# rrwick/Filtlong

Measured on NVIDIA H100. Metric: Gbases/sec scored+filtered, higher is better.
Workload: dtype f64

## Files before the change

### filtlong_b200/csrc/fl_phred.cu

```cuda
#include "fl_device.cuh"

namespace {

#define PH_THREADS 256
#define PH_SMEM (256 * 8 * 16 + 256 * 16 * 8)
#define PH_SEG 16384
#define PH_LONG (PH_SEG + PH_SEG / 2)

#define ITEM_FUSED 0xFFFFFFFFu
#define ITEM_MEAN 0xFFFFFFFEu

struct Tab {
    const double2 *tqa;
    const double *ta;
};

struct PhredArgs {
    const uint8_t *qual;
    const uint64_t *off;
    const int32_t *len;
    uint32_t n;
    const double *lut;
    fl_params p;
    int32_t *r_len, *r_first, *r_last, *r_nbad, *r_nchild;
    double *r_mean, *r_window;
    uint8_t *r_passed;
    unsigned long long *r_rowstart;
    uint32_t *w_parent;
    int32_t *w_start, *w_end;
    double *w_mean, *w_window;
    uint8_t *w_passed;
    unsigned long long read_base, row_base;
    const unsigned long long *item_start;
    const uint32_t *order;
    const uint2 *items;
    unsigned long long n_items;
    double *it_a, *it_b, *it_c;
    uint32_t *fallback;
    unsigned long long *work;
    unsigned long long *phred_paths;
    int head_len;
};

__device__ __forceinline__ unsigned byte_of(uint32_t w, int i) { return (w >> (8 * i)) & 0xFFu; }

template <int WI>
__device__ __forceinline__ void out_words(const uint4 &a, const uint4 &b, unsigned sh, uint32_t ow[4]) {
    const uint32_t c[8] = {a.x, a.y, a.z, a.w, b.x, b.y, b.z, b.w};
#pragma unroll
    for (int k = 0; k < 4; ++k) ow[k] = __funnelshift_r(c[WI + k], c[WI + k + 1], sh);
}

template <bool DO_SUM, bool DO_WIN>
__device__ __forceinline__ void step(unsigned cin, unsigned cout, const Tab &t, double &sum, double &w, double &best) {
    if (DO_SUM && DO_WIN) {
        const double2 qa = t.tqa[cin * 8];
        const double ao = t.ta[cout * 16];
        sum += qa.x;
        w -= ao;
        w += qa.y;
        if (w < best) best = w;
    } else if (DO_SUM) {
        sum += t.tqa[cin * 8].x;
    } else {
        const double ai = t.ta[cin * 16];
        const double ao = t.ta[cout * 16];
        w -= ao;
        w += ai;
        if (w < best) best = w;
    }
}

template <bool DO_SUM, bool DO_WIN>
__device__ __forceinline__ void chain(const uint8_t *__restrict__ q, int jlo, int jhi, int ws, const Tab &t, double &sum,
                                      double &w, double &best) {
    int j = jlo;
    for (; (j & 15) && j < jhi; ++j) step<DO_SUM, DO_WIN>(q[j], DO_WIN ? q[j - ws] : 0u, t, sum, w, best);
    if (j + 16 <= jhi) {
        const uint4 *qv = reinterpret_cast<const uint4 *>(q);
        const uint4 zero = make_uint4(0u, 0u, 0u, 0u);
        int blk = 0;
        unsigned sh = 0, wi = 0;
        uint4 oa = zero, ob = zero;
        if (DO_WIN) {
            const int i0 = j - ws;
            blk = i0 >> 4;
            sh = ((unsigned)i0 & 3u) * 8u;
            wi = ((unsigned)i0 & 15u) >> 2;
            oa = __ldg(qv + blk);
            ob = __ldg(qv + blk + 1);
        }
        uint4 in = __ldg(qv + (j >> 4));
        while (j + 16 <= jhi) {
            const bool more = j + 32 <= jhi;
            const uint4 in_next = more ? __ldg(qv + (j >> 4) + 1) : zero;
            const uint4 oc = (DO_WIN && more) ? __ldg(qv + blk + 2) : zero;
            uint32_t ow[4] = {0u, 0u, 0u, 0u};
            if (DO_WIN) {
                switch (wi) {
                    case 0: out_words<0>(oa, ob, sh, ow); break;
                    case 1: out_words<1>(oa, ob, sh, ow); break;
                    case 2: out_words<2>(oa, ob, sh, ow); break;
                    default: out_words<3>(oa, ob, sh, ow); break;
                }
            }
            const uint32_t iw[4] = {in.x, in.y, in.z, in.w};
#pragma unroll
            for (int k = 0; k < 4; ++k)
#pragma unroll
                for (int b = 0; b < 4; ++b)
                    step<DO_SUM, DO_WIN>(byte_of(iw[k], b), byte_of(ow[k], b), t, sum, w, best);
            in = in_next;
            oa = ob;
            ob = oc;
            ++blk;
            j += 16;
        }
    }
    for (; j < jhi; ++j) step<DO_SUM, DO_WIN>(q[j], DO_WIN ? q[j - ws] : 0u, t, sum, w, best);
}

__device__ __forceinline__ void write_read(const PhredArgs &a, uint32_t r, int L, double mean, double window) {
    const uint8_t passed = fl_hard_cutoffs(a.p, L, mean, window);
    a.r_len[r] = L;
    a.r_mean[r] = mean;
    a.r_window[r] = window;
    a.r_passed[r] = passed;
    a.r_first[r] = -1;
    a.r_last[r] = -1;
    a.r_nbad[r] = 0;
    a.r_nchild[r] = 0;
    a.r_rowstart[r] = a.row_base + r;
    a.w_parent[r] = (uint32_t)(a.read_base + r);
    a.w_start[r] = 0;
    a.w_end[r] = L;
    a.w_mean[r] = mean;
    a.w_window[r] = window;
    a.w_passed[r] = passed;
}

__device__ __forceinline__ void finish(const PhredArgs &a, uint32_t r, int L, double sum, double best) {
    const double wsd = (double)a.p.window_size;
    if (best < 0.5 / wsd) best = 0.0;
    write_read(a, r, L, 100.0 * sum / (double)L, 100.0 * best);
}

__device__ __forceinline__ void score_fused(const PhredArgs &a, uint32_t r, const Tab &t) {
    const int L = a.len[r], ws = a.p.window_size;
    const uint8_t *q = a.qual + a.off[r];
    double sum = 0.0, w = 0.0, best = 0.0;
    chain<true, false>(q, 0, L < ws ? L : ws, ws, t, sum, w, best);
    if (L <= ws) {
        const double mean = 100.0 * sum / (double)L;
        write_read(a, r, L, mean, mean);
        return;
    }
    w = sum / (double)ws;
    best = w;
    chain<true, true>(q, ws, L, ws, t, sum, w, best);
    finish(a, r, L, sum, best);
}

__device__ __forceinline__ int n_segments(int L, int ws) { return (L - ws + PH_SEG - 1) / PH_SEG; }

__device__ __forceinline__ unsigned long long items_of(int L, int ws) {
    if (L <= PH_LONG || L <= ws + PH_SEG) return 1ull;
    return 1ull + (unsigned long long)n_segments(L, ws);
}

__device__ __forceinline__ void score_segment(const PhredArgs &a, uint32_t r, int seg, size_t idx, const Tab &t) {
    const int L = a.len[r], ws = a.p.window_size;
    const uint8_t *q = a.qual + a.off[r];
    double sum = 0.0, w = 0.0, best = 0.0;
    chain<true, false>(q, 0, ws, ws, t, sum, w, best);
    const double w0 = sum / (double)ws;
    const int P = ws + seg * PH_SEG;
    const int Pend = (P + PH_SEG < L) ? P + PH_SEG : L;
    double entry = w0;
    if (seg > 0) {
        int e = 0;
        (void)frexp(w0, &e);
        const double scale = ldexp(1.0, 53 - e);
        long long s0 = 0, sp = 0;
        for (int i = 0; i < ws; ++i) {
            s0 += __double2ll_rn(t.ta[(unsigned)q[i] * 16] * scale);
            sp += __double2ll_rn(t.ta[(unsigned)q[P - ws + i] * 16] * scale);
        }
        entry = w0 + (double)(sp - s0) / scale;
    }
    w = entry;
    best = __longlong_as_double(0x7FF0000000000000ll);
    chain<false, true>(q, P, Pend, ws, t, sum, w, best);
    a.it_a[idx] = entry;
    a.it_b[idx] = w;
    a.it_c[idx] = best;
}

__device__ __forceinline__ Tab make_tables(const double *lut, unsigned char *smem_raw) {
    double2 *tqa_all = reinterpret_cast<double2 *>(smem_raw);
    double *ta_all = reinterpret_cast<double *>(smem_raw + 256 * 8 * 16);
    for (int i = threadIdx.x; i < 256 * 8; i += blockDim.x) {
        const int c = i >> 3;
        tqa_all[i] = make_double2(lut[c], lut[256 + c]);
    }
    for (int i = threadIdx.x; i < 256 * 16; i += blockDim.x) ta_all[i] = lut[256 + (i >> 4)];
    __syncthreads();
    const unsigned lane = threadIdx.x & 31;
    Tab t;
    t.tqa = tqa_all + (lane & 7);
    t.ta = ta_all + (lane & 15);
    return t;
}

__global__ void __launch_bounds__(PH_THREADS, 3) k_phred_items(PhredArgs a) {
    extern __shared__ __align__(16) unsigned char smem_raw[];
    const Tab t = make_tables(a.lut, smem_raw);
    const size_t T = (size_t)gridDim.x * blockDim.x;
    for (size_t it = (size_t)blockIdx.x * blockDim.x + threadIdx.x; it < a.n_items; it += T) {
        const size_t idx = a.order[it];
        const uint2 item = a.items[idx];
        const uint32_t r = item.x;
        if (item.y == ITEM_FUSED) {
            score_fused(a, r, t);
        } else if (item.y == ITEM_MEAN) {
            continue;
        } else {
            score_segment(a, r, (int)item.y, idx, t);
        }
    }
}

#define PH_MEAN_SMEM (256 * 16 * 8)
#define PH_MEAN_TILE 2048

__device__ __forceinline__ double serial_tile(const uint8_t *__restrict__ q, int lo, int hi, const double *__restrict__ qtab,
                                              double s) {
    for (int j = lo; j < hi; ++j) s += __ldg(qtab + (unsigned)q[j]);
    return s;
}

__global__ void __launch_bounds__(256) k_phred_mean_long(PhredArgs a, unsigned long long tie_binades) {
    extern __shared__ __align__(16) unsigned char smem_raw[];
    double *qtab_all = reinterpret_cast<double *>(smem_raw);
    for (int i = threadIdx.x; i < 256 * 16; i += blockDim.x) {
        const double v = a.lut[i >> 4];
        qtab_all[i] = (v >= 0.0 && v < 1.0) ? v : __longlong_as_double(0x7FF8000000000000ll);
    }
    __syncthreads();
    const unsigned lane = threadIdx.x & 31;
    const double *qtab = qtab_all + (lane & 15);
    const size_t warp = ((size_t)blockIdx.x * blockDim.x + threadIdx.x) >> 5, n_warps = ((size_t)gridDim.x * blockDim.x) >> 5;
    for (size_t r = warp; r < a.n; r += n_warps) {
        const size_t base = a.item_start[r];
        if (a.item_start[r + 1] - base <= 1) continue;
        const int L = a.len[r];
        const uint8_t *q = a.qual + a.off[r];
        const uint4 *qv = reinterpret_cast<const uint4 *>(q);
        double s = 0.0;
        int j = 0, small_left = 0;
        while (j < L) {
            int e = -2000;
            if (s > 0.0) {
                (void)frexp(s, &e);
                e -= 1;
            }
            const bool big = e >= 10 && e <= 1000 && small_left == 0;
            const bool lattice_ok = big || (e >= 6 && e <= 1000);
            const int T = big ? PH_MEAN_TILE : 128;
            const int hi = (j + T < L) ? j + T : L;
            bool done = false;
            if (lattice_ok) {
                const double C = ldexp(1.0, e), half_ulp = ldexp(1.0, e - 53);
                const bool check_ties = e < 64 && ((tie_binades >> e) & 1ull);
                double d = 0.0;
                unsigned bad = 0u;
#pragma unroll
                for (int c4 = 0; c4 < 4; ++c4) {
                    const int lo = j + 512 * c4 + 16 * (int)lane;
                    if (lo < hi) {
                        const uint4 v = __ldg(qv + (lo >> 4));
                        const uint32_t wv[4] = {v.x, v.y, v.z, v.w};
                        if (lo + 16 <= hi && !check_ties) {
#pragma unroll
                            for (int k = 0; k < 16; ++k) {
                                const double x = qtab[byte_of(wv[k >> 2], k & 3) * 16];
                                d += (C + x) - C;
                            }
                        } else {
#pragma unroll
                            for (int k = 0; k < 16; ++k) {
                                const double x = qtab[byte_of(wv[k >> 2], k & 3) * 16];
                                const double rq = (C + x) - C;
                                const bool in = lo + k < hi;
                                bad |= (in && fabs(x - rq) == half_ulp) ? 1u : 0u;
                                d += in ? rq : 0.0;
                            }
                        }
                    }
                }
#pragma unroll
                for (int o = 16; o; o >>= 1) {
                    d += __shfl_xor_sync(0xffffffffu, d, o);
                    bad |= __shfl_xor_sync(0xffffffffu, bad, o);
                }
                if (!bad) {
                    const double s_new = s + d;
                    if (s_new < C + C) { s = s_new; done = true; }
                }
            }
            if (!done) {
                if (big) { small_left = PH_MEAN_TILE / 128; continue; }
                if (lane == 0) s = serial_tile(q, j, hi, a.lut, s);
                s = __shfl_sync(0xffffffffu, s, 0);
            }
            if (small_left > 0) --small_left;
            j = hi;
        }
        if (lane == 0) a.it_a[base] = s;
    }
}

__global__ void __launch_bounds__(256) k_phred_merge(PhredArgs a) {
    const uint32_t r = blockIdx.x * blockDim.x + threadIdx.x;
    if (r >= a.n) return;
    const size_t base = a.item_start[r];
    const int n_it = (int)(a.item_start[r + 1] - base);
    if (n_it <= 1) return;
    const int L = a.len[r];
    const double sum = a.it_a[base];
    double best = a.it_a[base + 1];
    bool ok = true;
    for (int k = 0; k < n_it - 1; ++k) {
        const size_t i = base + 1 + k;
        if (k > 0 && __double_as_longlong(a.it_a[i]) != __double_as_longlong(a.it_b[i - 1])) { ok = false; break; }
        const double b = a.it_c[i];
        if (b < best) best = b;
    }
    if (ok) finish(a, r, L, sum, best);
    else a.fallback[1 + atomicAdd(a.fallback, 1u)] = r;
}

__global__ void __launch_bounds__(PH_THREADS, 3) k_phred_fallback(PhredArgs a) {
    extern __shared__ __align__(16) unsigned char smem_raw[];
    const uint32_t n = a.fallback[0];
    if (n == 0) return;
    const Tab t = make_tables(a.lut, smem_raw);
    for (size_t i = (size_t)blockIdx.x * blockDim.x + threadIdx.x; i < n; i += (size_t)gridDim.x * blockDim.x)
        score_fused(a, a.fallback[1 + i], t);
}

__global__ void k_phred_plan(const int32_t *__restrict__ len, uint32_t n, int ws, unsigned long long *__restrict__ n_items) {
    const uint32_t r = blockIdx.x * blockDim.x + threadIdx.x;
    if (r < n) n_items[r] = items_of(len[r], ws);
}

__global__ void k_phred_fill(const int32_t *__restrict__ len, uint32_t n, int ws, const unsigned long long *__restrict__ item_start,
                             uint2 *__restrict__ items, uint32_t *__restrict__ cost) {
    const uint32_t r = blockIdx.x * blockDim.x + threadIdx.x;
    if (r >= n) return;
    const int L = len[r];
    const size_t base = item_start[r];
    const int cnt = (int)items_of(L, ws);
    if (cnt == 1) {
        items[base] = make_uint2(r, ITEM_FUSED);
        cost[base] = 0 * 256 + fl_length_bucket(L);
        return;
    }
    items[base] = make_uint2(r, ITEM_MEAN);
    cost[base] = 2 * 256 + fl_length_bucket(L);
    for (int k = 0; k < cnt - 1; ++k) {
        items[base + 1 + k] = make_uint2(r, (uint32_t)k);
        const int P = ws + k * PH_SEG;
        cost[base + 1 + k] = 1 * 256 + fl_length_bucket(((P + PH_SEG < L) ? PH_SEG : L - P) + 2 * ws);
    }
}

#define PT_THREADS 256
#define PT_SMEM (256 * 16 * 8)
#define PS_TILE 512
#define PS_OCC 3

struct TieInfo {
    unsigned long long any;
    unsigned long long many;
    unsigned char ch[64];
};

__device__ __forceinline__ int exponent_of(double v) { return (int)((__double2hiint(v) >> 20) & 0x7FF) - 1023; }
__device__ __forceinline__ double pow2(int e) { return __hiloint2double((e + 1023) << 20, 0); }
__device__ __forceinline__ double shfl_d(double v, int src) { return __shfl_sync(0xffffffffu, v, src); }

__device__ __forceinline__ long long warp_incl_scan_ll(long long v, unsigned lane) {
#pragma unroll
    for (int d = 1; d < 32; d <<= 1) {
        const long long t = __shfl_up_sync(0xffffffffu, v, d);
        if (lane >= (unsigned)d) v += t;
    }
    return v;
}
__device__ __forceinline__ long long warp_sum_ll(long long v) {
#pragma unroll
    for (int o = 16; o; o >>= 1) v += __shfl_xor_sync(0xffffffffu, v, o);
    return v;
}

template <int COPIES = 16, typename T>
__device__ __forceinline__ const T *entry_of(const T *tl, uint32_t w, int k) {
    const uint32_t c = __byte_perm(w, 0u, 0x4440u + (unsigned)k);
    return reinterpret_cast<const T *>(reinterpret_cast<const unsigned char *>(tl) + c * (unsigned)(COPIES * sizeof(T)));
}

__global__ void __launch_bounds__(PH_THREADS, 3) k_phred_first(PhredArgs a) {
    extern __shared__ __align__(16) unsigned char smem_raw[];
    const Tab t = make_tables(a.lut, smem_raw);
    const int ws = a.p.window_size;
    for (size_t r = (size_t)blockIdx.x * blockDim.x + threadIdx.x; r < a.n; r += (size_t)gridDim.x * blockDim.x) {
        const int L = a.len[r];
        const uint8_t *q = a.qual + a.off[r];
        double sum = 0.0, w = 0.0, best = 0.0;
        chain<true, false>(q, 0, L < ws ? L : ws, ws, t, sum, w, best);
        if (L <= ws) {
            const double mean = 100.0 * sum / (double)L;
            write_read(a, (uint32_t)r, L, mean, mean);
            continue;
        }
        a.it_b[r] = sum / (double)ws;
        chain<true, false>(q, ws, L < a.head_len ? L : a.head_len, ws, t, sum, w, best);
        a.it_a[r] = sum;
    }
}

template <int NW>
__device__ __forceinline__ bool chunk_has(const uint32_t (&cw)[NW], unsigned ch) {
    const uint32_t pat = ch * 0x01010101u;
    uint32_t hit = 0;
#pragma unroll
    for (int i = 0; i < NW; ++i) hit |= __vcmpeq4(cw[i], pat);
    return hit != 0u;
}

__global__ void __launch_bounds__(PT_THREADS, PS_OCC) k_phred_sum(PhredArgs a, TieInfo tie) {
    extern __shared__ __align__(16) unsigned char smem_raw[];
    double *tab = reinterpret_cast<double *>(smem_raw);
    __shared__ TieInfo s_tie;
    const double qnan = __longlong_as_double(0x7FF8000000000000ll);
    if (threadIdx.x == 0) s_tie = tie;
    for (int i = threadIdx.x; i < 256 * 16; i += blockDim.x) {
        const double q = a.lut[i >> 4];
        tab[i] = (q >= 0.0 && q < 1.0) ? q : qnan;
    }
    __syncthreads();
    const unsigned lane = threadIdx.x & 31;
    const double *tl = tab + (lane & 15);
    const int H = a.head_len;
    const float inv_tile = 1.0f / (float)PS_TILE;
    for (;;) {
        unsigned long long it = 0;
        if (lane == 0) it = atomicAdd(a.work + 0, 1ull);
        it = __shfl_sync(0xffffffffu, it, 0);
        if (it >= a.n) break;
        const uint32_t r = a.order[it];
        const int L = a.len[r];
        if (L <= H) continue;
        const uint8_t *q = a.qual + a.off[r];
        const uint4 *qv = reinterpret_cast<const uint4 *>(q);
        double s0 = a.it_a[r];
        long long sb = __double_as_longlong(s0);
        int e = exponent_of(s0);
        double Cs = pow2(e), acc = Cs;
        int budget = 0;
        bool tieflag = e >= 0 && e < 64 && ((s_tie.any >> e) & 1ull);
        bool nanf = false;
        uint4 pre = make_uint4(0x21212121u, 0x21212121u, 0x21212121u, 0x21212121u);
        if (H + 16 * (int)lane < L) pre = __ldg(qv + ((H >> 4) + (int)lane));
        for (int j = H; j < L; j += PS_TILE) {
            uint32_t cw[4] = {pre.x, pre.y, pre.z, pre.w};
            {
                const int pn = j + PS_TILE + 16 * (int)lane;
                if (pn < L) pre = __ldg(qv + (pn >> 4));
            }
            const int n = (L - j < PS_TILE) ? L - j : PS_TILE;
            if (n < PS_TILE) {
                const int nv = n - 16 * (int)lane;
#pragma unroll
                for (int i = 0; i < 4; ++i) {
                    const int vb = nv - 4 * i;
                    const uint32_t m = vb >= 4 ? 0xFFFFFFFFu : (vb <= 0 ? 0u : (0xFFFFFFFFu >> (32 - 8 * vb)));
                    cw[i] = (cw[i] & m) | (0x21212121u & ~m);
                }
            }
            const bool in_range = e >= 5 && e < 52;
            int mode = 0;
            if (budget == 0 || tieflag) {
                if (budget == 0) {
                    nanf |= (acc != acc);
                    sb += warp_sum_ll(__double_as_longlong(acc) - __double_as_longlong(Cs));
                    acc = Cs;
                    if (in_range) {
                        long long room = ((__double_as_longlong(Cs) + (1ll << 52)) - sb) >> (52 - e);
                        if (room > (1ll << 30)) room = 1ll << 30;
                        budget = room >= 1 ? (int)((room - 1) >> 9) : 0;
                    }
                }
                if (!in_range || sb <= 0) {
                    mode = 2;
                } else {
                    if (tieflag && (((s_tie.many >> e) & 1ull) || __any_sync(0xffffffffu, chunk_has<4>(cw, s_tie.ch[e])))) mode = 2;
                    if (mode == 2 && budget > 0) {
                        sb += warp_sum_ll(__double_as_longlong(acc) - __double_as_longlong(Cs));
                        acc = Cs;
                        budget = 0;
                    }
                    if (mode == 0 && budget == 0) mode = 1;
                }
            }
#pragma unroll
            for (int k = 0; k < 16; ++k) acc += *entry_of(tl, cw[k >> 2], k & 3);
            if (mode == 0) {
                --budget;
                continue;
            }
            bool serial = mode == 2 || __any_sync(0xffffffffu, acc != acc);
            if (!serial) {
                long long cur = sb;
                int ce = e, lo = 0;
                double C = Cs, part = acc;
                for (int round = 0; round < 6; ++round) {
                    const long long top = __double_as_longlong(C) + (1ll << 52);
                    const long long u = (int)lane >= lo ? __double_as_longlong(part) - __double_as_longlong(C) : 0ll;
                    const long long P = warp_incl_scan_ll(u, lane);
                    const unsigned cross = __ballot_sync(0xffffffffu, cur + P >= top);
                    if (cross == 0u) {
                        sb = cur + __shfl_sync(0xffffffffu, P, 31);
                        e = ce;
                        Cs = C;
                        break;
                    }
                    const int lx = __ffs(cross) - 1;
                    const double t0 = __longlong_as_double(cur + __shfl_sync(0xffffffffu, P - u, lx));
                    C = C + C;
                    ce += 1;
                    double v = (int)lane == lx ? t0 : C;
                    if ((int)lane >= lx) {
#pragma unroll
                        for (int k = 0; k < 16; ++k) v += *entry_of(tl, cw[k >> 2], k & 3);
                    }
                    const double t = shfl_d(v, lx);
                    bool hit = false;
                    if ((s_tie.any >> ce) & 1ull) hit = ((s_tie.many >> ce) & 1ull) || __any_sync(0xffffffffu, chunk_has<4>(cw, s_tie.ch[ce]));
                    if (hit || exponent_of(t) != ce || !(t == t) || round == 5) {
                        serial = true;
                        break;
                    }
                    cur = __double_as_longlong(t);
                    lo = lx + 1;
                    part = v;
                }
                if (!serial) tieflag = (s_tie.any >> e) & 1ull;
            }
            if (serial) {
                double v = __longlong_as_double(sb);
                if (lane == 0)
                    for (int p = 0; p < n; ++p) v += __ldg(a.lut + (unsigned)q[j + p]);
                v = shfl_d(v, 0);
                sb = __double_as_longlong(v);
                e = exponent_of(v);
                Cs = pow2(e);
                tieflag = e >= 0 && e < 64 && ((s_tie.any >> e) & 1ull);
            }
            acc = Cs;
            budget = 0;
        }
        nanf |= (acc != acc);
        sb += warp_sum_ll(__double_as_longlong(acc) - __double_as_longlong(Cs));
        const bool any_nan = __any_sync(0xffffffffu, nanf);
        if (lane == 0) a.it_a[r] = any_nan ? qnan : __longlong_as_double(sb);
    }
}

template <int NW>
__device__ __forceinline__ void load_raw(const uint32_t *__restrict__ q32, int pos, int maxword, uint32_t (&w)[NW + 1]) {
    const int wi = pos >> 2;
#pragma unroll
    for (int i = 0; i <= NW; ++i) {
        const int x = wi + i;
        w[i] = __ldg(q32 + (x < maxword ? x : maxword));
    }
}
template <int NW>
__device__ __forceinline__ void align_raw(const uint32_t (&w)[NW + 1], int pos, uint32_t (&o)[NW]) {
    const unsigned bs = ((unsigned)pos & 3u) * 8u;
#pragma unroll
    for (int i = 0; i < NW; ++i) o[i] = __funnelshift_r(w[i], w[i + 1], bs);
}

#define PT_ANCHOR 0.75
#define PT_ANCHOR_BITS 0x3FE8000000000000ll
#define PW_SHIFT 30
#define PW_BAD 0x800000u
#define PW_NONE 0xFFFFFFFFu
#define PW_CHUNK 2048
#define PW_SMEM (256 * 32 * 4 + 256 * 8 * 8)
enum { PW_CAND = 0, PW_FULL = 1, PW_BAD_BYTE = 2, PW_LOW = 3, PW_COUNTERS = 9 };

__device__ __forceinline__ void prefetch_chunk(const uint8_t *q, int pos, int padded) {
    if (pos >= padded) return;
    const int end = pos + PW_CHUNK < padded ? pos + PW_CHUNK : padded;
    asm volatile("cp.async.bulk.prefetch.L2.global [%0], %1;" ::"l"(q + pos), "r"((uint32_t)(end - pos)) : "memory");
}

__device__ __forceinline__ uint32_t warp_incl_scan_u32(uint32_t v) {
#pragma unroll
    for (int d = 1; d < 32; d <<= 1)
        asm("{\n\t.reg .u32 t;\n\t.reg .pred p;\n\t"
            "shfl.sync.up.b32 t|p, %0, %1, 0, 0xffffffff;\n\t"
            "@p add.u32 %0, %0, t;\n\t}"
            : "+r"(v) : "r"(d));
    return v;
}

template <int K, bool TAIL>
__device__ __forceinline__ void win_core(const uint32_t (&cw)[(K + 3) / 4], const uint32_t (&cwas)[(K + 3) / 4],
                                         const double *__restrict__ tl, int nvalid, double &x, double &m) {
    x = PT_ANCHOR;
    m = PT_ANCHOR;
#pragma unroll
    for (int k = 0; k < K; ++k) {
        if (!TAIL || k < nvalid) {
            const double now = *entry_of<8>(tl, cw[k >> 2], k & 3), was = *entry_of<8>(tl, cwas[k >> 2], k & 3);
            x += now - was;
            m = x < m ? x : m;
        }
    }
}

template <int K, bool TAIL>
__device__ __forceinline__ void filter_core(const uint32_t (&cw)[(K + 3) / 4], uint32_t fbase, int nvalid,
                                            const uint32_t (&was)[K], uint32_t (&now)[K], int &x, int &m) {
    x = 0;
    m = 0;
#pragma unroll
    for (int k = 0; k < K; ++k) {
        const uint32_t c = __byte_perm(cw[k >> 2], 0u, 0x4440u + (unsigned)(k & 3));
        asm volatile("ld.shared.u32 %0, [%1];" : "=r"(now[k]) : "r"(fbase + (c << 7)));
        if (!TAIL || k < nvalid) {
            x += (int)(now[k] - was[k]);
            m = min(m, x);
        }
    }
}

template <int K>
__device__ __forceinline__ long long window_grid(const uint32_t *__restrict__ q32, int pos, int maxword, const double *__restrict__ tg,
                                                 const uint32_t (&keep)[(K + 3) / 4], const uint32_t (&fill)[(K + 3) / 4],
                                                 uint32_t (&cw)[(K + 3) / 4]) {
    constexpr int NW = (K + 3) / 4;
    uint32_t raw[NW + 1];
    load_raw<NW>(q32, pos, maxword, raw);
    align_raw<NW>(raw, pos, cw);
    double s = 0.0;
#pragma unroll
    for (int i = 0; i < NW; ++i) cw[i] = (cw[i] & keep[i]) | fill[i];
#pragma unroll
    for (int k = 0; k < K; ++k) s += *entry_of<8>(tg, cw[k >> 2], k & 3);
    return warp_sum_ll(__double2ll_rn(s * 9007199254740992.0));
}

template <int K>
__device__ __forceinline__ long long win_exact(const uint32_t *__restrict__ q32, int maxword, int L, int ws, int t0, int t1,
                                               long long W0b, const double *__restrict__ tg, int lpos, int nb_lane,
                                               const uint32_t (&keep)[(K + 3) / 4], const uint32_t (&fill)[(K + 3) / 4],
                                               unsigned lane) {
    constexpr int NW = (K + 3) / 4;
    uint32_t cwas[NW];
    const long long S0 = window_grid<K>(q32, lpos, maxword, tg, keep, fill, cwas);
    long long Wb = W0b + (window_grid<K>(q32, t0 * ws + lpos, maxword, tg, keep, fill, cwas) - S0);
    long long mnb = 0x7FFFFFFFFFFFFFFFll;
    const int jend = min(L, ws + t1 * ws);
    uint32_t pre[NW + 1];
    load_raw<NW>(q32, ws + t0 * ws + lpos, maxword, pre);
    for (int j = ws + t0 * ws; j < jend; j += ws) {
        uint32_t cw[NW];
        align_raw<NW>(pre, j + lpos, cw);
        if (j + ws < jend) load_raw<NW>(q32, j + ws + lpos, maxword, pre);
        const int n = L - j;
        double x, m;
        if (n >= ws) {
#pragma unroll
            for (int i = 0; i < NW; ++i) cw[i] = (cw[i] & keep[i]) | fill[i];
            win_core<K, false>(cw, cwas, tg, K, x, m);
        } else {
            win_core<K, true>(cw, cwas, tg, max(0, min(nb_lane, n - lpos)), x, m);
        }
        const long long nx = __double_as_longlong(x) - PT_ANCHOR_BITS;
        const long long inc = warp_incl_scan_ll(nx, lane);
        const long long cand = Wb + (inc - nx) + (__double_as_longlong(m) - PT_ANCHOR_BITS);
        mnb = cand < mnb ? cand : mnb;
        Wb += __shfl_sync(0xffffffffu, inc, 31);
#pragma unroll
        for (int i = 0; i < NW; ++i) cwas[i] = cw[i];
    }
    return mnb;
}

template <int K>
__global__ void __launch_bounds__(PT_THREADS, 4) k_phred_win(PhredArgs a) {
    constexpr int NW = (K + 3) / 4;
    extern __shared__ __align__(16) unsigned char smem_raw[];
    uint32_t *ftab = reinterpret_cast<uint32_t *>(smem_raw);
    double *gtab = reinterpret_cast<double *>(smem_raw + 256 * 32 * 4);
    __shared__ double s_amax;
    __shared__ uint32_t s_mask[32][4];
    const int ws = a.p.window_size;
    const double qnan = __longlong_as_double(0x7FF8000000000000ll);
    if (threadIdx.x == 0) {
        double mx = 0.0;
        for (int c = 0; c < 256; ++c) {
            const double v = a.lut[256 + c];
            if (v >= 0.0 && v > mx && v * (double)ws <= 1.0 - 1e-10) mx = v;
        }
        s_amax = (0.5 + mx) - 0.5;
    }
    if (threadIdx.x < 32) {
        const int nb = max(0, min(K, ws - K * (int)threadIdx.x));
        for (int i = 0; i < 2; ++i) {
            uint32_t m = 0;
            for (int b = 0; b < 4; ++b)
                if (4 * i + b < nb) m |= 0xFFu << (8 * b);
            s_mask[threadIdx.x][i] = m;
            s_mask[threadIdx.x][2 + i] = 0x21212121u & ~m;
        }
    }
    for (int i = threadIdx.x; i < 256 * 32; i += blockDim.x) {
        const double v = a.lut[256 + (i >> 5)];
        bool ok = v >= 0.0 && v * (double)ws <= 1.0 - 1e-10;
        if (ok && v > 0.0) {
            const double sc = ldexp(v, 53);
            ok = (sc - floor(sc)) != 0.5;
        }
        const double g = (0.5 + v) - 0.5;
        ftab[i] = ok ? (uint32_t)(__double2ull_rn(ldexp(g, 53)) >> PW_SHIFT) : PW_BAD;
        if ((i & 31) < 8) gtab[(i >> 5) * 8 + (i & 31)] = ok ? g : qnan;
    }
    __syncthreads();
    const unsigned lane = threadIdx.x & 31;
    const uint32_t fbase = (uint32_t)__cvta_generic_to_shared(ftab + lane);
    const double *tg = gtab + (lane & 7);
    const double thr = 0.5 + 2.0 * s_amax;
    const int nb_lane = max(0, min(K, ws - K * (int)lane));
    const int lpos = K * (int)lane;
    uint32_t keep[NW], fill[NW];
#pragma unroll
    for (int i = 0; i < NW; ++i) {
        keep[i] = s_mask[lane][i];
        fill[i] = s_mask[lane][2 + i];
    }
    unsigned long long paths = 0;
    for (;;) {
        unsigned long long it = 0;
        if (lane == 0) it = atomicAdd(a.work + 1, 1ull);
        it = __shfl_sync(0xffffffffu, it, 0);
        if (it >= a.n) break;
        const uint32_t r = a.order[it];
        const int L = a.len[r];
        if (L <= ws) continue;
        const uint8_t *q = a.qual + a.off[r];
        const uint32_t *q32 = reinterpret_cast<const uint32_t *>(q);
        const int padded = (L + 63) & ~63;
        const int maxword = (padded >> 2) - 1;
        const int nsteps = (L - 1) / ws;
        const double W0 = a.it_b[r];
        bool reject = !(W0 >= thr && W0 < 1.0);
        uint32_t best = PW_NONE, other = PW_NONE, S0f = 0;
        int bstep = 0;
        if (!reject) {
            uint32_t va[K], vb[K];
            {
                uint32_t raw[NW + 1], cw[NW];
                load_raw<NW>(q32, lpos, maxword, raw);
                align_raw<NW>(raw, lpos, cw);
#pragma unroll
                for (int k = 0; k < K; ++k) {
                    va[k] = (k < nb_lane) ? ftab[__byte_perm(cw[k >> 2], 0u, 0x4440u + (unsigned)(k & 3)) * 32 + lane] : 0u;
                    S0f += va[k];
                }
            }
            S0f = __reduce_add_sync(0xffffffffu, S0f);
            uint32_t W = S0f;
            reject = W >= PW_BAD;
            uint32_t pre[NW + 1];
            if (lane == 0) {
                prefetch_chunk(q, 0, padded);
                prefetch_chunk(q, PW_CHUNK, padded);
            }
            int pf = 2 * PW_CHUNK;
            load_raw<NW>(q32, ws + lpos, maxword, pre);
            int j = ws, t = 0;
#define PW_STEP(WAS, NOW)                                                                                     \
            {                                                                                                 \
                uint32_t cw[NW];                                                                              \
                if (j + ws > pf - PW_CHUNK) {         \
                    if (lane == 0) prefetch_chunk(q, pf, padded);                                             \
                    pf += PW_CHUNK;                                                                           \
                }                                                                                             \
                align_raw<NW>(pre, j + lpos, cw);                                                             \
                if (j + ws < L) load_raw<NW>(q32, j + ws + lpos, maxword, pre);                               \
                const int n = L - j;                                                                          \
                int x, m;                                                                                     \
                if (n >= ws) {                                                                                \
                    _Pragma("unroll") for (int i = 0; i < NW; ++i) cw[i] = (cw[i] & keep[i]) | fill[i];       \
                    filter_core<K, false>(cw, fbase, K, WAS, NOW, x, m);                                      \
                } else {                                                                                      \
                    filter_core<K, true>(cw, fbase, max(0, min(nb_lane, n - lpos)), WAS, NOW, x, m);          \
                }                                                                                             \
                const uint32_t inc = warp_incl_scan_u32((uint32_t)x);                                         \
                const uint32_t cand = W + (inc - (uint32_t)x) + (uint32_t)m;                                  \
                other = min(other, max(cand, best));                                                          \
                bstep = cand < best ? t : bstep;                                                              \
                best = min(best, cand);                                                                       \
                W += __shfl_sync(0xffffffffu, inc, 31);                                                       \
                reject |= W >= PW_BAD;                                                                        \
                j += ws;                                                                                      \
                ++t;                                                                                          \
            }
            while (!reject) {
                PW_STEP(va, vb)
                if (j >= L || reject) break;
                PW_STEP(vb, va)
                if (j >= L) break;
            }
#undef PW_STEP
        }
        const double s = a.it_a[r];
        double mn = 0.0;
        int path = PW_BAD_BYTE, exact_steps = 0;
        if (!reject) {
            const uint32_t mt = min(__reduce_min_sync(0xffffffffu, best), S0f);
            const bool rel = best <= mt + (uint32_t)ws;
            const bool ambiguous = __any_sync(0xffffffffu, rel && other <= best + (uint32_t)ws);
            uint32_t pend = ambiguous ? (lane == 0 ? 0u : PW_NONE) : (rel ? (uint32_t)bstep : PW_NONE);
            long long mnb = __double_as_longlong(W0);
            for (;;) {
                const uint32_t t = __reduce_min_sync(0xffffffffu, pend);
                if (t == PW_NONE) break;
                const int t1 = ambiguous ? nsteps : (int)t + 1;
                const long long c = win_exact<K>(q32, maxword, L, ws, (int)t, t1, __double_as_longlong(W0), tg, lpos, nb_lane, keep, fill, lane);
                mnb = c < mnb ? c : mnb;
                exact_steps += t1 - (int)t;
                if (pend == t) pend = PW_NONE;
            }
#pragma unroll
            for (int o = 16; o; o >>= 1) {
                const long long v = __shfl_xor_sync(0xffffffffu, mnb, o);
                mnb = v < mnb ? v : mnb;
            }
            mn = __longlong_as_double(mnb);
            reject = !(mn >= thr) || !(s == s);
            path = reject ? PW_LOW : ambiguous ? PW_FULL : PW_CAND;
        }
        if (lane == 0) {
            if (reject) a.fallback[1 + atomicAdd(a.fallback, 1u)] = r;
            else finish(a, r, L, s, mn);
        }
        if (lane == 2u * path) paths += 1;
        else if (lane == 2u * path + 1) paths += (unsigned long long)L;
        else if (lane == 8) paths += (unsigned long long)exact_steps;
    }
    if (lane < PW_COUNTERS && paths) atomicAdd(a.phred_paths + lane, paths);
}

}

static int ensure_lut(fl_ctx *ctx) {
    if (ctx->d_lut && ctx->lut_window == ctx->p.window_size) return FL_OK;
    double h[512];
    fl_phred_luts(ctx->p.window_size, h, h + 256);
    if (!ctx->d_lut) FL_CUDA(ctx, cudaMalloc(&ctx->d_lut, sizeof(h)));
    FL_CUDA(ctx, cudaMemcpyAsync(ctx->d_lut, h, sizeof(h), cudaMemcpyHostToDevice, ctx->stream));
    ctx->tie_binades = 0;
    ctx->tie_many = 0;
    memset(ctx->tie_char, 0, sizeof(ctx->tie_char));
    for (int e = 0; e < 64; ++e)
        for (int c = 0; c < 256; ++c) {
            const double q = h[c];
            if (!(q > 0.0 && q < 1.0)) continue;
            const double scaled = ldexp(q, 52 - e);
            if (scaled - floor(scaled) == 0.5) {
                if (ctx->tie_binades & (1ull << e)) ctx->tie_many |= 1ull << e;
                ctx->tie_binades |= 1ull << e;
                ctx->tie_char[e] = (unsigned char)c;
            }
        }
    ctx->tie_binades_a = 0;
    for (int e = 0; e < 64; ++e)
        for (int c = 0; c < 256; ++c) {
            const double v = h[256 + c];
            if (!(v > 0.0 && v < 1.0)) continue;
            const double scaled = ldexp(v, 52 + e);
            if (scaled < 9007199254740992.0 && scaled - floor(scaled) == 0.5) ctx->tie_binades_a |= 1ull << e;
        }
    FL_CUDA(ctx, cudaStreamSynchronize(ctx->stream));
    ctx->lut_window = ctx->p.window_size;
    return FL_OK;
}

static int phred_args_of(fl_ctx *ctx, const BatchView &b, const PhredOut &o, PhredArgs *out) {
    PhredArgs a{};
    a.qual = b.qual; a.off = b.off; a.len = b.len; a.n = b.n;
    a.lut = ctx->d_lut; a.p = ctx->p;
    a.r_mean = o.mean; a.r_window = o.window; a.r_passed = o.passed;
    if (o.whole_reads) {
        const size_t rb = ctx->n_reads, wb = ctx->n_rows;
        a.r_len = ctx->r_len.p + rb; a.r_first = ctx->r_first.p + rb; a.r_last = ctx->r_last.p + rb;
        a.r_nbad = ctx->r_nbad.p + rb; a.r_nchild = ctx->r_nchild.p + rb;
        a.r_rowstart = ctx->r_rowstart.p + rb;
        a.w_parent = ctx->w_parent.p + wb; a.w_start = ctx->w_start.p + wb; a.w_end = ctx->w_end.p + wb;
        a.w_mean = ctx->w_mean.p + wb; a.w_window = ctx->w_window.p + wb; a.w_passed = ctx->w_passed.p + wb;
        a.read_base = rb; a.row_base = wb;
    } else {
        FL_CUDA(ctx, ctx->sc_sink.reserve((size_t)b.n + 1, 0, ctx->stream));
        unsigned long long *s = ctx->sc_sink.p;
        int32_t *s32 = reinterpret_cast<int32_t *>(s);
        a.r_len = a.r_first = a.r_last = a.r_nbad = a.r_nchild = a.w_start = a.w_end = s32;
        a.r_rowstart = s;
        a.w_parent = reinterpret_cast<uint32_t *>(s);
        a.w_mean = a.w_window = reinterpret_cast<double *>(s);
        a.w_passed = reinterpret_cast<uint8_t *>(s);
    }
    *out = a;
    return FL_OK;
}

int fl_score_phred(fl_ctx *ctx, const BatchView &b) {
    if (!b.qual) {
        ctx->set_error("FASTA input not supported without an external reference (no quality string and the k-mer set is empty)");
        return FL_EINVAL;
    }
    const size_t n = b.n;
    FL_TRY(fl_reserve_reads(ctx, ctx->n_reads + n));
    FL_TRY(fl_reserve_rows(ctx, ctx->n_rows + n));
    const size_t rb = ctx->n_reads;
    FL_TRY(fl_phred_pass(ctx, b, PhredOut{ctx->r_mean.p + rb, ctx->r_window.p + rb, ctx->r_passed.p + rb, true}));
    ctx->n_reads += n;
    ctx->n_rows += n;
    return FL_OK;
}

int fl_phred_pass(fl_ctx *ctx, const BatchView &b, const PhredOut &o) {
    FL_TRY(ensure_lut(ctx));
    const size_t n = b.n;
    cudaStream_t st = ctx->stream;
    const int ws = ctx->p.window_size;
    if (ctx->phred_mode != 0 && ws >= 16 && ws <= 256) {
        FL_CUDA(ctx, ctx->sc_order.reserve(n, 0, st));
        FL_TRY(fl_order_by_length(ctx, b.len, n, ctx->sc_order.p));
        PhredArgs a;
        FL_TRY(phred_args_of(ctx, b, o, &a));
        a.order = ctx->sc_order.p;
        a.head_len = (ws + 15) & ~15;
        FL_CUDA(ctx, ctx->sc_f64.reserve(3 * n + 8, 0, st));
        a.it_a = ctx->sc_f64.p; a.it_b = ctx->sc_f64.p + n; a.it_c = ctx->sc_f64.p + 2 * n;
        FL_CUDA(ctx, ctx->sc_u32a.reserve(n + 2, 0, st));
        a.fallback = ctx->sc_u32a.p;
        FL_CUDA(ctx, cudaMemsetAsync(a.fallback, 0, sizeof(uint32_t), st));
        a.work = ctx->d_scalars + 24;
        FL_CUDA(ctx, cudaMemsetAsync(a.work, 0, 2 * sizeof(unsigned long long), st));
        a.phred_paths = ctx->d_scalars + FL_SCALAR_PHRED_PATHS;
        if (!ctx->phred_attr_set) {
            FL_CUDA(ctx, cudaFuncSetAttribute(k_phred_sum, cudaFuncAttributeMaxDynamicSharedMemorySize, PT_SMEM));
            FL_CUDA(ctx, cudaFuncSetAttribute(k_phred_win<2>, cudaFuncAttributeMaxDynamicSharedMemorySize, PW_SMEM));
            FL_CUDA(ctx, cudaFuncSetAttribute(k_phred_win<4>, cudaFuncAttributeMaxDynamicSharedMemorySize, PW_SMEM));
            FL_CUDA(ctx, cudaFuncSetAttribute(k_phred_win<8>, cudaFuncAttributeMaxDynamicSharedMemorySize, PW_SMEM));
            FL_CUDA(ctx, cudaFuncSetAttribute(k_phred_first, cudaFuncAttributeMaxDynamicSharedMemorySize, PH_SMEM));
            FL_CUDA(ctx, cudaFuncSetAttribute(k_phred_fallback, cudaFuncAttributeMaxDynamicSharedMemorySize, PH_SMEM));
            ctx->phred_attr_set = true;
        }
        {
            unsigned hb = fl_blocks(n, PH_THREADS);
            if (hb > (unsigned)ctx->sm_count * 3) hb = (unsigned)ctx->sm_count * 3;
            k_phred_first<<<hb, PH_THREADS, PH_SMEM, st>>>(a);
            ctx->launches++;
        }
        const bool occ_set = ctx->phred_occupancy >= 1 && ctx->phred_occupancy <= 6;
        const unsigned want = fl_blocks(n * 32, PT_THREADS);
        const unsigned sblocks = min(want, (unsigned)ctx->sm_count * (unsigned)(occ_set ? ctx->phred_occupancy : PS_OCC));
        const unsigned blocks = min(want, (unsigned)ctx->sm_count * (unsigned)(occ_set ? ctx->phred_occupancy : 4));
        {
            KernelTimer kt(ctx, FL_KERNEL_SCORE_PHRED);
            TieInfo ti;
            ti.any = ctx->tie_binades;
            ti.many = ctx->tie_many;
            memcpy(ti.ch, ctx->tie_char, 64);
            k_phred_sum<<<sblocks, PT_THREADS, PT_SMEM, st>>>(a, ti);
            if (ws <= 64) k_phred_win<2><<<blocks, PT_THREADS, PW_SMEM, st>>>(a);
            else if (ws <= 128) k_phred_win<4><<<blocks, PT_THREADS, PW_SMEM, st>>>(a);
            else k_phred_win<8><<<blocks, PT_THREADS, PW_SMEM, st>>>(a);
            ctx->launches += 2;
        }
        k_phred_fallback<<<ctx->sm_count, PH_THREADS, PH_SMEM, st>>>(a);
        ctx->launches++;
        FL_CUDA(ctx, cudaGetLastError());
        return FL_OK;
    }
    FL_CUDA(ctx, ctx->sc_u64a.reserve(n + 1, 0, st));
    k_phred_plan<<<fl_blocks(n, 256), 256, 0, st>>>(b.len, b.n, ws, ctx->sc_u64a.p);
    ctx->launches++;
    FL_TRY(fl_exclusive_scan_u64(ctx, ctx->sc_u64a.p, ctx->sc_u64a.p, n, ctx->d_scalars));
    FL_CUDA(ctx, cudaMemcpyAsync(ctx->sc_u64a.p + n, ctx->d_scalars, sizeof(unsigned long long), cudaMemcpyDeviceToDevice, st));
    FL_CUDA(ctx, cudaMemcpyAsync(ctx->h_scalars, ctx->d_scalars, sizeof(unsigned long long), cudaMemcpyDeviceToHost, st));
    FL_CUDA(ctx, cudaStreamSynchronize(st));
    const size_t n_items = (size_t)ctx->h_scalars[0];
    FL_CUDA(ctx, ctx->sc_u64b.reserve(n_items + 1, 0, st));
    FL_CUDA(ctx, ctx->sc_u32a.reserve(n_items + n + 2, 0, st));
    FL_CUDA(ctx, ctx->sc_order.reserve(n_items, 0, st));
    FL_CUDA(ctx, ctx->sc_f64.reserve(3 * n_items + 8, 0, st));
    uint2 *items = reinterpret_cast<uint2 *>(ctx->sc_u64b.p);
    uint32_t *cost = ctx->sc_u32a.p;
    uint32_t *fallback = ctx->sc_u32a.p + n_items;
    k_phred_fill<<<fl_blocks(n, 256), 256, 0, st>>>(b.len, b.n, ws, ctx->sc_u64a.p, items, cost);
    ctx->launches++;
    FL_CUDA(ctx, cudaMemsetAsync(fallback, 0, sizeof(uint32_t), st));
    FL_TRY(fl_order_by_key(ctx, cost, n_items, ctx->sc_order.p));

    PhredArgs a;
    FL_TRY(phred_args_of(ctx, b, o, &a));
    a.item_start = ctx->sc_u64a.p; a.order = ctx->sc_order.p; a.items = items; a.n_items = n_items;
    a.it_a = ctx->sc_f64.p; a.it_b = ctx->sc_f64.p + n_items; a.it_c = ctx->sc_f64.p + 2 * n_items;
    a.fallback = fallback;
    if (!ctx->phred_items_attr_set) {
        FL_CUDA(ctx, cudaFuncSetAttribute(k_phred_items, cudaFuncAttributeMaxDynamicSharedMemorySize, PH_SMEM));
        FL_CUDA(ctx, cudaFuncSetAttribute(k_phred_fallback, cudaFuncAttributeMaxDynamicSharedMemorySize, PH_SMEM));
        ctx->phred_items_attr_set = true;
    }
    unsigned blocks = fl_blocks(n_items, PH_THREADS);
    const unsigned max_blocks = (unsigned)ctx->sm_count * 3;
    if (blocks > max_blocks) blocks = max_blocks;
    {
        KernelTimer kt(ctx, FL_KERNEL_SCORE_PHRED);
        k_phred_items<<<blocks, PH_THREADS, PH_SMEM, st>>>(a);
    }
    ctx->launches++;
    if (n_items > n) {
        k_phred_mean_long<<<ctx->sm_count * 6, 256, PH_MEAN_SMEM, st>>>(a, ctx->tie_binades);
        ctx->launches++;
        k_phred_merge<<<fl_blocks(n, 256), 256, 0, st>>>(a);
        k_phred_fallback<<<ctx->sm_count, PH_THREADS, PH_SMEM, st>>>(a);
        ctx->launches += 2;
    }
    FL_CUDA(ctx, cudaGetLastError());
    return FL_OK;
}
```

Before: 825.0.

## Pack per-read phred state into length-ordered records and prefetch next read

Adds a 32-byte per-read record (offset, length, read id, initial window, running sum) that the first kernel writes at the read's slot in length order, using a new inverse-permutation kernel. The sum and window kernels then claim records with one coalesced warp load instead of chasing order/len/off/it_a/it_b through scattered gathers. They also stop at the highest live slot instead of scanning all reads, and issue an L2 bulk prefetch for the next read's qualities. The head length is raised to at least 1024 so that more of each read is summed in the per-thread first pass. In exchange it adds an extra kernel launch and memory, and relies on the records and slot bounds staying consistent; the sum kernel also holds an empty chunk-boundary check.

```diff
diff --git a/filtlong_b200/csrc/fl_phred.cu b/filtlong_b200/csrc/fl_phred.cu
--- a/filtlong_b200/csrc/fl_phred.cu
+++ b/filtlong_b200/csrc/fl_phred.cu
@@ -13,6 +13,14 @@
 struct Tab {
     const double2 *tqa;
     const double *ta;
+};
+
+struct __align__(32) PhredRec {
+    unsigned long long off;
+    int32_t len;
+    uint32_t r;
+    double w0;
+    double sum;
 };
 
 struct PhredArgs {
@@ -36,8 +44,11 @@
     const uint2 *items;
     unsigned long long n_items;
     double *it_a, *it_b, *it_c;
+    PhredRec *rec;
+    const uint32_t *slot_of;
     uint32_t *fallback;
     unsigned long long *work;
+    unsigned long long *ends;
     unsigned long long *phred_paths;
     int head_len;
 };
@@ -380,6 +391,13 @@
 #define PS_TILE 512
 #define PS_OCC 3
 
+#define PW_CHUNK 2048
+__device__ __forceinline__ void prefetch_chunk(const uint8_t *q, int pos, int padded) {
+    if (pos >= padded) return;
+    const int end = pos + PW_CHUNK < padded ? pos + PW_CHUNK : padded;
+    asm volatile("cp.async.bulk.prefetch.L2.global [%0], %1;" ::"l"(q + pos), "r"((uint32_t)(end - pos)) : "memory");
+}
+
 struct TieInfo {
     unsigned long long any;
     unsigned long long many;
@@ -410,24 +428,68 @@
     return reinterpret_cast<const T *>(reinterpret_cast<const unsigned char *>(tl) + c * (unsigned)(COPIES * sizeof(T)));
 }
 
+__global__ void k_phred_slots(const uint32_t *__restrict__ order, uint32_t n, uint32_t *__restrict__ slot_of) {
+    const uint32_t it = blockIdx.x * blockDim.x + threadIdx.x;
+    if (it < n) slot_of[order[it]] = it;
+}
+
 __global__ void __launch_bounds__(PH_THREADS, 3) k_phred_first(PhredArgs a) {
     extern __shared__ __align__(16) unsigned char smem_raw[];
     const Tab t = make_tables(a.lut, smem_raw);
     const int ws = a.p.window_size;
-    for (size_t r = (size_t)blockIdx.x * blockDim.x + threadIdx.x; r < a.n; r += (size_t)gridDim.x * blockDim.x) {
-        const int L = a.len[r];
-        const uint8_t *q = a.qual + a.off[r];
-        double sum = 0.0, w = 0.0, best = 0.0;
-        chain<true, false>(q, 0, L < ws ? L : ws, ws, t, sum, w, best);
-        if (L <= ws) {
-            const double mean = 100.0 * sum / (double)L;
-            write_read(a, (uint32_t)r, L, mean, mean);
-            continue;
-        }
-        a.it_b[r] = sum / (double)ws;
-        chain<true, false>(q, ws, L < a.head_len ? L : a.head_len, ws, t, sum, w, best);
-        a.it_a[r] = sum;
-    }
+    const unsigned lane = threadIdx.x & 31;
+    const size_t stride = (size_t)gridDim.x * blockDim.x;
+    for (size_t r0 = (size_t)blockIdx.x * blockDim.x + (threadIdx.x & ~31u); r0 < a.n; r0 += stride) {
+        const uint32_t r = (uint32_t)(r0 + lane);
+        uint32_t live_sum = 0, live_win = 0;
+        if (r < a.n) {
+            const uint32_t it = a.slot_of[r];
+            const int L = a.len[r];
+            const unsigned long long off = a.off[r];
+            const uint8_t *q = a.qual + off;
+            double sum = 0.0, w = 0.0, best = 0.0, w0;
+            chain<true, false>(q, 0, L < ws ? L : ws, ws, t, sum, w, best);
+            if (L <= ws) {
+                const double mean = 100.0 * sum / (double)L;
+                write_read(a, r, L, mean, mean);
+                w0 = sum;
+            } else {
+                w0 = sum / (double)ws;
+                chain<true, false>(q, ws, L < a.head_len ? L : a.head_len, ws, t, sum, w, best);
+                live_win = it + 1u;
+                live_sum = L > a.head_len ? it + 1u : 0u;
+            }
+            PhredRec rec;
+            rec.off = off;
+            rec.len = L;
+            rec.r = r;
+            rec.w0 = w0;
+            rec.sum = sum;
+            a.rec[it] = rec;
+        }
+        live_sum = __reduce_max_sync(0xffffffffu, live_sum);
+        live_win = __reduce_max_sync(0xffffffffu, live_win);
+        if (lane == 0 && live_sum) atomicMax(a.ends + 0, (unsigned long long)live_sum);
+        if (lane == 0 && live_win) atomicMax(a.ends + 1, (unsigned long long)live_win);
+    }
+}
+
+__device__ __forceinline__ uint32_t claim_record(const PhredArgs &a, unsigned long long *ctr, unsigned long long bound, unsigned lane) {
+    unsigned long long it = 0;
+    if (lane == 0) it = atomicAdd(ctr, 1ull);
+    it = __shfl_sync(0xffffffffu, it, 0);
+    if (it >= bound) return 0xFFFFFFFFu;
+    return lane < 8 ? __ldg(reinterpret_cast<const uint32_t *>(a.rec + it) + lane) : (uint32_t)it;
+}
+__device__ __forceinline__ uint32_t rec_word(uint32_t nxt, int k) { return __shfl_sync(0xffffffffu, nxt, k); }
+__device__ __forceinline__ unsigned long long rec_off(uint32_t nxt) {
+    return ((unsigned long long)rec_word(nxt, 1) << 32) | rec_word(nxt, 0);
+}
+__device__ __forceinline__ double rec_f64(uint32_t nxt, int k) { return __hiloint2double((int)rec_word(nxt, k + 1), (int)rec_word(nxt, k)); }
+__device__ __forceinline__ void prefetch_next(const PhredArgs &a, uint32_t nxt, int thr, unsigned lane) {
+    const unsigned long long off = rec_off(nxt);
+    const int L = (int)rec_word(nxt, 2);
+    if (lane == 0 && L > thr) prefetch_chunk(a.qual + off, 0, (L + 63) & ~63);
 }
 
 template <int NW>
@@ -454,17 +516,18 @@
     const double *tl = tab + (lane & 15);
     const int H = a.head_len;
     const float inv_tile = 1.0f / (float)PS_TILE;
+    const unsigned long long bound = a.ends[0];
+    uint32_t nxt = claim_record(a, a.work + 0, bound, lane);
     for (;;) {
-        unsigned long long it = 0;
-        if (lane == 0) it = atomicAdd(a.work + 0, 1ull);
-        it = __shfl_sync(0xffffffffu, it, 0);
-        if (it >= a.n) break;
-        const uint32_t r = a.order[it];
-        const int L = a.len[r];
+        const int L = (int)rec_word(nxt, 2);
+        if (L < 0) break;
+        const uint32_t it = rec_word(nxt, 8);
+        const uint8_t *q = a.qual + rec_off(nxt);
+        const double s0 = rec_f64(nxt, 6);
+        nxt = claim_record(a, a.work + 0, bound, lane);
+        nxt = lane == 9 ? it : nxt;
         if (L <= H) continue;
-        const uint8_t *q = a.qual + a.off[r];
         const uint4 *qv = reinterpret_cast<const uint4 *>(q);
-        double s0 = a.it_a[r];
         long long sb = __double_as_longlong(s0);
         int e = exponent_of(s0);
         double Cs = pow2(e), acc = Cs;
@@ -473,7 +536,11 @@
         bool nanf = false;
         uint4 pre = make_uint4(0x21212121u, 0x21212121u, 0x21212121u, 0x21212121u);
         if (H + 16 * (int)lane < L) pre = __ldg(qv + ((H >> 4) + (int)lane));
-        for (int j = H; j < L; j += PS_TILE) {
+        int j = H;
+        for (; j < L; j += PS_TILE) {
+            const int c = (j + PS_TILE - 1) / PW_CHUNK;
+            if (c != (j - 1) / PW_CHUNK) {
+            }
             uint32_t cw[4] = {pre.x, pre.y, pre.z, pre.w};
             {
                 const int pn = j + PS_TILE + 16 * (int)lane;
@@ -574,7 +641,8 @@
         nanf |= (acc != acc);
         sb += warp_sum_ll(__double_as_longlong(acc) - __double_as_longlong(Cs));
         const bool any_nan = __any_sync(0xffffffffu, nanf);
-        if (lane == 0) a.it_a[r] = any_nan ? qnan : __longlong_as_double(sb);
+        const uint32_t it_done = rec_word(nxt, 9);
+        if (lane == 0) a.rec[it_done].sum = any_nan ? qnan : __longlong_as_double(sb);
     }
 }
 
@@ -599,15 +667,8 @@
 #define PW_SHIFT 30
 #define PW_BAD 0x800000u
 #define PW_NONE 0xFFFFFFFFu
-#define PW_CHUNK 2048
 #define PW_SMEM (256 * 32 * 4 + 256 * 8 * 8)
 enum { PW_CAND = 0, PW_FULL = 1, PW_BAD_BYTE = 2, PW_LOW = 3, PW_COUNTERS = 9 };
-
-__device__ __forceinline__ void prefetch_chunk(const uint8_t *q, int pos, int padded) {
-    if (pos >= padded) return;
-    const int end = pos + PW_CHUNK < padded ? pos + PW_CHUNK : padded;
-    asm volatile("cp.async.bulk.prefetch.L2.global [%0], %1;" ::"l"(q + pos), "r"((uint32_t)(end - pos)) : "memory");
-}
 
 __device__ __forceinline__ uint32_t warp_incl_scan_u32(uint32_t v) {
 #pragma unroll
@@ -756,25 +817,32 @@
         fill[i] = s_mask[lane][2 + i];
     }
     unsigned long long paths = 0;
+    const unsigned long long bound = a.ends[1];
+    uint32_t nxt = claim_record(a, a.work + 1, bound, lane);
     for (;;) {
-        unsigned long long it = 0;
-        if (lane == 0) it = atomicAdd(a.work + 1, 1ull);
-        it = __shfl_sync(0xffffffffu, it, 0);
-        if (it >= a.n) break;
-        const uint32_t r = a.order[it];
-        const int L = a.len[r];
+        const int L = (int)rec_word(nxt, 2);
+        if (L < 0) break;
+        const uint32_t r = rec_word(nxt, 3);
+        const uint8_t *q = a.qual + rec_off(nxt);
+        const double W0 = rec_f64(nxt, 4);
+        const double s = rec_f64(nxt, 6);
+        nxt = claim_record(a, a.work + 1, bound, lane);
         if (L <= ws) continue;
-        const uint8_t *q = a.qual + a.off[r];
         const uint32_t *q32 = reinterpret_cast<const uint32_t *>(q);
         const int padded = (L + 63) & ~63;
         const int maxword = (padded >> 2) - 1;
         const int nsteps = (L - 1) / ws;
-        const double W0 = a.it_b[r];
         bool reject = !(W0 >= thr && W0 < 1.0);
         uint32_t best = PW_NONE, other = PW_NONE, S0f = 0;
         int bstep = 0;
         if (!reject) {
             uint32_t va[K], vb[K];
+            if (lane == 0) {
+                prefetch_chunk(q, 0, padded);
+                prefetch_chunk(q, PW_CHUNK, padded);
+            }
+            uint32_t pre[NW + 1];
+            load_raw<NW>(q32, ws + lpos, maxword, pre);
             {
                 uint32_t raw[NW + 1], cw[NW];
                 load_raw<NW>(q32, lpos, maxword, raw);
@@ -788,13 +856,7 @@
             S0f = __reduce_add_sync(0xffffffffu, S0f);
             uint32_t W = S0f;
             reject = W >= PW_BAD;
-            uint32_t pre[NW + 1];
-            if (lane == 0) {
-                prefetch_chunk(q, 0, padded);
-                prefetch_chunk(q, PW_CHUNK, padded);
-            }
             int pf = 2 * PW_CHUNK;
-            load_raw<NW>(q32, ws + lpos, maxword, pre);
             int j = ws, t = 0;
 #define PW_STEP(WAS, NOW)                                                                                     \
             {                                                                                                 \
@@ -831,7 +893,7 @@
             }
 #undef PW_STEP
         }
-        const double s = a.it_a[r];
+        prefetch_next(a, nxt, ws, lane);
         double mn = 0.0;
         int path = PW_BAD_BYTE, exact_steps = 0;
         if (!reject) {
@@ -957,11 +1019,16 @@
         PhredArgs a;
         FL_TRY(phred_args_of(ctx, b, o, &a));
         a.order = ctx->sc_order.p;
-        a.head_len = (ws + 15) & ~15;
-        FL_CUDA(ctx, ctx->sc_f64.reserve(3 * n + 8, 0, st));
-        a.it_a = ctx->sc_f64.p; a.it_b = ctx->sc_f64.p + n; a.it_c = ctx->sc_f64.p + 2 * n;
-        FL_CUDA(ctx, ctx->sc_u32a.reserve(n + 2, 0, st));
+        a.head_len = max((ws + 15) & ~15, 1024);
+        FL_CUDA(ctx, ctx->sc_f64.reserve(4 * n + 8, 0, st));
+        a.rec = reinterpret_cast<PhredRec *>(ctx->sc_f64.p);
+        a.ends = reinterpret_cast<unsigned long long *>(ctx->sc_f64.p + 4 * n);
+        FL_CUDA(ctx, cudaMemsetAsync(a.ends, 0, 2 * sizeof(unsigned long long), st));
+        FL_CUDA(ctx, ctx->sc_u32a.reserve(2 * n + 2, 0, st));
         a.fallback = ctx->sc_u32a.p;
+        a.slot_of = ctx->sc_u32a.p + n + 2;
+        k_phred_slots<<<fl_blocks(n, 256), 256, 0, st>>>(a.order, (uint32_t)n, ctx->sc_u32a.p + n + 2);
+        ctx->launches++;
         FL_CUDA(ctx, cudaMemsetAsync(a.fallback, 0, sizeof(uint32_t), st));
         a.work = ctx->d_scalars + 24;
         FL_CUDA(ctx, cudaMemsetAsync(a.work, 0, 2 * sizeof(unsigned long long), st));
```

New measurement: 867.3 (median of 6 runs). 1.05x the previous value.
